# Insomnia34/charon

Measured on AMD Instinct MI355X. Metric: verified BLS partial sigs/sec (node) + threshold aggregates/sec, 1/2/4/8 GPU, higher is better.
Workload: dtype u32

## Files before the change

charon_amd/csrc/ops.h:

```cpp
#pragma once
#include "../../include/hipbls.h"
#include "fr.h"
#include "h2c.h"
#include "pairing.h"
#include "pairing_lds.h"

namespace bls {

BLS_HD BLS_CALL bool pairing_check_verify(const g1a& pk, const g2a& hm, const g2a& sig) {
  g1a P[2];
  g2a Q[2];
  bool skip[2] = {false, false};
  P[0] = pk;
  Q[0] = hm;
  P[1].x = G1_GEN_X;
  P[1].y = G1_NEG_GEN_Y;
  Q[1] = sig;
  fp12 f, e;
  miller_loop_n(f, P, Q, skip, 2);
  final_exponentiation(e, f);
  return fp12_is_one(e);
}

BLS_HD BLS_CALL int pairing_check_verify_sig(const g1a& pk, const g2a& hm, const g2a& sig) {
  g1a P1;
  P1.x = G1_GEN_X;
  P1.y = G1_NEG_GEN_Y;
  fp12 f, e;
  g2j T1;
  miller_loop_2(f, pk, hm, P1, sig, &T1);
  const bool in_g2 = g2_subgroup_from_miller(T1, sig);
  final_exponentiation(e, f);
  if (!in_g2) return HIPBLS_ERR_SIGNATURE;
  return fp12_is_one(e) ? HIPBLS_OK : HIPBLS_ERR_VERIFY;
}

#ifndef BLS_VERIFY_L_CALL
#define BLS_VERIFY_L_CALL BLS_CALL
#endif
template <int S, bool INL, bool LINES = false>
BLS_HD BLS_INLINE int pairing_check_verify_sig_l_body(const g1a& pk, const g2a& hm, const g2a& sig, const f12l<S> F,
                                                    const rl_plan* plan = nullptr) {
  g1a P1;
  P1.x = G1_GEN_X;
  P1.y = G1_NEG_GEN_Y;
  fp12 f;
  bool in_g2;
  {
    g2j T1;
    if (LINES) {
      bool done = false;
      if (rl_wave_all(plan->replay != nullptr)) {
        done = miller_loop_2_l_replay<S>(f, F, pk, sig, &T1, plan->replay, plan->seed);
        rl_count(plan->lctr, RL_CTR_HITS, done);
        rl_count(plan->lctr, RL_CTR_BAD, !done);
      }
      if (!done && rl_wave_any(plan->record != nullptr)) {
        rl_recorder rec{plan->record, plan->seed};
        miller_loop_2_l_body<S, true>(f, F, pk, hm, P1, sig, &T1, rec);
        if (plan->record) {
          rl_publish(*plan, rec.h);
          rl_count(plan->lctr, RL_CTR_PUBLISHED, true);
        }
      } else if (!done) {
        miller_loop_2_l_body<S, true>(f, F, pk, hm, P1, sig, &T1);
      }
    } else if (INL)
      miller_loop_2_l_body<S, true>(f, F, pk, hm, P1, sig, &T1);
    else
      miller_loop_2_l<S, true>(f, F, pk, hm, P1, sig, &T1);
    in_g2 = g2_subgroup_from_miller(T1, sig);
  }
  final_exp_l(f, f, F);
  if (!in_g2) return HIPBLS_ERR_SIGNATURE;
  return fp12_is_one(f) ? HIPBLS_OK : HIPBLS_ERR_VERIFY;
}
template <int S>
BLS_HD BLS_VERIFY_L_CALL int pairing_check_verify_sig_l(const g1a& pk, const g2a& hm, const g2a& sig, const f12l<S> F) {
  return pairing_check_verify_sig_l_body<S, false>(pk, hm, sig, F);
}

BLS_HD BLS_INLINE int verify_inf_status(int ds, const g2a& sig) {
  if (ds == DEC_OK) {
    g2j sj;
    jac_from_aff(sj, sig);
    if (!g2_in_subgroup(sj)) return HIPBLS_ERR_SIGNATURE;
  }
  return HIPBLS_ERR_VERIFY;
}




BLS_HD BLS_CALL void lagrange_at_zero(fr& out_plain, const int64_t* ids, int n, int i) {
  fr num, den, t, xi, xj;
  fr_from_u32(num, 1);
  fr_from_u32(den, 1);
  fr_from_i64(xi, ids[i]);
  for (int j = 0; j < n; ++j) {
    if (j == i) continue;
    fr_from_i64(xj, ids[j]);
    fr_mul(num, num, xj);
    fr_sub(t, xj, xi);
    fr_mul(den, den, t);
  }
  fr_inv(den, den);
  fr_mul(t, num, den);
  fr_to_plain(out_plain, t);
}

BLS_HD BLS_INLINE uint64_t gcd_u64(uint64_t a, uint64_t b) {
  while (b) {
    const uint64_t t = a % b;
    a = b;
    b = t;
  }
  return a;
}
BLS_HD BLS_CALL bool lagrange_small(const int64_t* ids, int t, int me, int64_t& c_me, uint64_t& L) {
  if (t < 1 || t > 16) return false;
  for (int a = 0; a < t; ++a)
    if (ids[a] > (1 << 20) || ids[a] < -(1 << 20) || ids[a] == 0) return false;
  int64_t D[16];
  uint64_t l = 1;
  for (int k = 0; k < t; ++k) {
    int64_t d = 1;
    for (int j = 0; j < t; ++j) {
      if (j == k) continue;
      if (__builtin_mul_overflow(d, ids[j] - ids[k], &d)) return false;
    }
    if (d == 0 || d == INT64_MIN) return false;
    D[k] = d;
    const uint64_t ad = d < 0 ? (uint64_t)(-d) : (uint64_t)d;
    if (__builtin_mul_overflow(l, ad / gcd_u64(l, ad), &l) || l > (uint64_t)INT64_MAX) return false;
  }
  for (int k = 0; k < t; ++k) {
    int64_t n = 1;
    for (int j = 0; j < t; ++j)
      if (j != k && __builtin_mul_overflow(n, ids[j], &n)) return false;
    const uint64_t ad = D[k] < 0 ? (uint64_t)(-D[k]) : (uint64_t)D[k];
    const int64_t f = D[k] < 0 ? -(int64_t)(l / ad) : (int64_t)(l / ad);
    int64_t c;
    if (__builtin_mul_overflow(n, f, &c) || c == INT64_MIN) return false;
    if (k == me) c_me = c;
  }
  L = l;
  return true;
}

BLS_HD BLS_INLINE void g2_mul_i64(g2j& r, const g2j& p, int64_t c) {
  jac_mul_u64(r, p, c < 0 ? (uint64_t)0 - (uint64_t)c : (uint64_t)c);
  if (c < 0) {
    g2j t = r;
    jac_neg(r, t);
  }
}

BLS_HD BLS_CALL void tagg_scale_point(g2j& out, const g2j& sj, const int64_t* ids, int t, int me) {
  int64_t c;
  uint64_t L;
  if (lagrange_small(ids, t, me, c, L)) {
    g2_mul_i64(out, sj, c);
  } else {
    fr lam;
    lagrange_at_zero(lam, ids, t, me);
    g2_mul_glv4(out, sj, lam.v);
  }
}

BLS_HD BLS_CALL bool g2_subgroup_and_mul_i64(g2j& out, const g2j& sj, int64_t c) {
  const uint64_t k = c < 0 ? (uint64_t)0 - (uint64_t)c : (uint64_t)c;
  g2j pw = sj, ax, ac;
  jac_set_inf(ax);
  jac_set_inf(ac);
  for (int i = 0; i < 64; ++i) {
    if ((X_ABS >> i) & 1ull) {
      g2j t = ax;
      jac_add(ax, t, pw);
    }
    if ((k >> i) & 1ull) {
      g2j t = ac;
      jac_add_body(ac, t, pw);
    }
    if (i < 63 && ((X_ABS | k) >> (i + 1)) != 0) {
      g2j t;
      jac_dbl_body(t, pw);
      pw = t;
    }
  }
  if (c < 0) {
    g2j t = ac;
    jac_neg(ac, t);
  }
  out = ac;
  g2j q, ps;
  jac_neg(q, ax);
  g2_psi(ps, sj);
  return jac_eq(q, ps);
}

BLS_HD BLS_CALL void tagg_unscale(g2j& acc, const int64_t* ids, int t) {
  int64_t c;
  uint64_t L;
  if (!lagrange_small(ids, t, 0, c, L) || jac_is_inf(acc)) return;
  fr lf, li, plain;
  fr_from_i64(lf, (int64_t)L);
  fr_inv(li, lf);
  fr_to_plain(plain, li);
  g2j x = acc;
  g2_mul_glv4(acc, x, plain.v);
}

BLS_HD BLS_INLINE uint64_t tagg_group_L(const int64_t* ids, int t) {
  int64_t c;
  uint64_t L;
  return lagrange_small(ids, t, 0, c, L) ? L : 1;
}
BLS_HD BLS_CALL void g1_scale_affine(g1a& pk, uint64_t L) {
  if (L <= 1) return;
  g1j pj, q;
  jac_from_aff(pj, pk);
  jac_mul_u64(q, pj, L);
  jac_to_aff(pk, q);
}

BLS_HD BLS_CALL int op_threshold_aggregate(uint8_t* out96, const uint8_t* sigs, const int64_t* ids, int t) {
  int st = t > 0 ? HIPBLS_OK : HIPBLS_ERR_COMBINE;
  for (int a = 0; a < t; ++a) {
    if (ids[a] == 0) st = HIPBLS_ERR_COMBINE;
    for (int b = a + 1; b < t; ++b)
      if (ids[a] == ids[b]) st = HIPBLS_ERR_COMBINE;
  }
  g2j acc;
  jac_set_inf(acc);
  for (int k = 0; k < t; ++k) {
    g2a s;
    const int ds = g2_decompress(s, sigs + 96 * k, true);
    if (ds == DEC_BAD) return HIPBLS_ERR_SIGNATURE;
    if (st != HIPBLS_OK || ds == DEC_INF) continue;
    g2j sj, p;
    jac_from_aff(sj, s);
    tagg_scale_point(p, sj, ids, t, k);
    g2j x = acc;
    jac_add(acc, x, p);
  }
  if (st != HIPBLS_OK) return st;
  tagg_unscale(acc, ids, t);
  g2_compress(out96, acc);
  return HIPBLS_OK;
}

BLS_HD BLS_CALL int op_verify(const uint8_t* pk48, const uint8_t* msg, uint32_t msg_len, const uint8_t* sig96) {
  g1a pk;
  const int dp = g1_decompress(pk, pk48, true);
  if (dp == DEC_BAD) return HIPBLS_ERR_PUBKEY;
  g2a sig;
  const int ds = g2_decompress(sig, sig96, false);
  if (ds == DEC_BAD) return HIPBLS_ERR_SIGNATURE;
  if (dp == DEC_INF || ds == DEC_INF) return verify_inf_status(ds, sig);
  g2j hj;
  hash_to_g2(hj, msg, msg_len, DST_POP, 43);
  g2a hm;
  jac_to_aff(hm, hj);
  return pairing_check_verify_sig(pk, hm, sig);
}

template <int S, bool INL>
BLS_HD BLS_INLINE int op_verify_l_rest(int dp, const g1a& pk, const uint8_t* msg, uint32_t msg_len,
                                       const uint8_t* sig96, const f12l<S> F) {
  if (dp == DEC_BAD) return HIPBLS_ERR_PUBKEY;
  g2a sig;
  const int ds = g2_decompress(sig, sig96, false);
  if (ds == DEC_BAD) return HIPBLS_ERR_SIGNATURE;
  if (dp == DEC_INF || ds == DEC_INF) return verify_inf_status(ds, sig);
  g2j hj;
  hash_to_g2(hj, msg, msg_len, DST_POP, 43);
  g2a hm;
  jac_to_aff(hm, hj);
  return pairing_check_verify_sig_l_body<S, INL>(pk, hm, sig, F);
}
template <int S, bool INL>
BLS_HD BLS_INLINE int op_verify_l_body(const uint8_t* pk48, const uint8_t* msg, uint32_t msg_len, const uint8_t* sig96,
                                     const f12l<S> F) {
  g1a pk;
  const int dp = g1_decompress(pk, pk48, true);
  return op_verify_l_rest<S, INL>(dp, pk, msg, msg_len, sig96, F);
}
template <int S>
BLS_HD BLS_VERIFY_L_CALL int op_verify_l(const uint8_t* pk48, const uint8_t* msg, uint32_t msg_len, const uint8_t* sig96,
                                const f12l<S> F) {
  return op_verify_l_body<S, false>(pk48, msg, msg_len, sig96, F);
}
template <int S>
BLS_HD BLS_INLINE int op_verify_l_kernel(const uint8_t* pk48, const uint8_t* msg, uint32_t msg_len, const uint8_t* sig96,
                                         const f12l<S> F) {
  return op_verify_l_body<S, true>(pk48, msg, msg_len, sig96, F);
}

BLS_HD BLS_CALL int op_sign(uint8_t* out96, const uint8_t* sk32, const uint8_t* msg, uint32_t msg_len) {
  fr sk;
  if (!fr_plain_from_be32(sk, sk32)) return HIPBLS_ERR_SECRET;
  g2j h, s;
  hash_to_g2(h, msg, msg_len, DST_POP, 43);
  g2_mul_glv4(s, h, sk.v);
  g2_compress(out96, s);
  return HIPBLS_OK;
}

BLS_HD BLS_CALL int op_sk_to_pk(uint8_t* out48, const uint8_t* sk32) {
  fr sk;
  if (!fr_plain_from_be32(sk, sk32)) return HIPBLS_ERR_SECRET;
  if (fr_is_zero(sk)) return HIPBLS_ERR_SECRET;
  g1j g, pk;
  g.x = G1_GEN_X;
  g.y = G1_GEN_Y;
  fp_set_one(g.z);
  jac_mul_limbs(pk, g, sk.v, 8);
  g1_compress(out48, pk);
  return HIPBLS_OK;
}

}
```

charon_amd/csrc/pairing_lds.h:

```cpp
#pragma once
#include "pairing.h"
#include "rootcache.h"

namespace bls {

#if defined(__HIP_DEVICE_COMPILE__)
#define BLS_LDS __attribute__((address_space(3)))
#else
#define BLS_LDS
#endif

typedef uint32_t u32x4 __attribute__((vector_size(16)));

template <int S>
struct f12l {
  BLS_LDS u32x4* p;

  BLS_HD BLS_MEMBER void ld_fp(fp& r, int g) const {
    for (int j = 0; j < 3; ++j) {
      const u32x4 q = p[(g + j) * S];
      r.v[4 * j] = q[0];
      r.v[4 * j + 1] = q[1];
      r.v[4 * j + 2] = q[2];
      r.v[4 * j + 3] = q[3];
// ... 215 lines not shown
  fp2_sub(c, s.c1, d.c1);
  F.st(4, c);
  fp2_sub(c, s.c2, d.c2);
  F.st(5, c);
}

template <class A>
BLS_HD BLS_INLINE void fp6_mul_01_fetch(fp6& r, const A& a, const fp2& b0, const fp2& b1) {
#if BLS_LAZY_FP6
  fp2 xa2, c0, c1, c2;
  fp2_mul_xi(xa2, a(2));
  fp2_mul2(c0, a(0), b0, xa2, b1);
  fp2_mul2(c1, a(0), b1, a(1), b0);
  fp2_mul2(c2, a(2), b0, a(1), b1);
  r.c0 = c0;
  r.c1 = c1;
  r.c2 = c2;
#else
  fp2 t0, t1, s0, s1, u, c0, c1, c2;
  fp2_mul(t0, a(0), b0);
  fp2_mul(t1, a(1), b1);
  fp2_mul(u, a(2), b1);
  fp2_mul_xi(u, u);
  fp2_add(c0, u, t0);
  fp2_add_lazy(s0, a(0), a(1));
  fp2_add(s1, b0, b1);
  fp2_mul(c1, s0, s1);
  fp2_sub(c1, c1, t0);
  fp2_sub(c1, c1, t1);
  fp2_mul(c2, a(2), b0);
  fp2_add(c2, c2, t1);
  r.c0 = c0;
  r.c1 = c1;
  r.c2 = c2;
#endif
}
template <class A>
BLS_HD BLS_INLINE void fp6_mul_1_fetch(fp6& r, const A& a, const fp2& b1) {
  fp2 c0;
  fp2_mul(c0, a(2), b1);
  fp2_mul_xi(r.c0, c0);
  fp2_mul(r.c1, a(0), b1);
  fp2_mul(r.c2, a(1), b1);
}

template <int S>
BLS_HD BLS_INLINE void fp12_mul_line_l(const f12l<S>& F, const fp2& g0_in, const fp2& g1_in, const fp2& h1_in) {
  const fp2 g0 = g0_in;
  const fp2 g1 = g1_in;
  const fp2 h1 = h1_in;
  fp6 t0, t1;
  fp6_mul_01_fetch(t0, [&](int i) { return F.ld(i); }, g0, g1);
  fp6_mul_1_fetch(t1, [&](int i) { return F.ld(3 + i); }, h1);
  fp2 c;
  for (int i = 0; i < 3; ++i) {
    fp2_add(c, F.ld(i), F.ld(3 + i));
    F.st(3 + i, c);
  }
  fp6 d;
  {
    fp6 vt1;
    fp6_mul_v(vt1, t1);
    fp2_add(c, t0.c0, vt1.c0);
    F.st(0, c);
    fp2_add(c, t0.c1, vt1.c1);
    F.st(1, c);
    fp2_add(c, t0.c2, vt1.c2);
    F.st(2, c);
    fp6_add(d, t0, t1);
  }
  fp2 gh1;
  fp2_add(gh1, g1, h1);
  fp6 s;
  fp6_mul_01_fetch(s, [&](int i) { return F.ld(3 + i); }, g0, gh1);
  fp2_sub(c, s.c0, d.c0);
  F.st(3, c);
  fp2_sub(c, s.c1, d.c1);
  F.st(4, c);
  fp2_sub(c, s.c2, d.c2);
  F.st(5, c);
}

#ifndef BLS_ML_PARK
#define BLS_ML_PARK 6
#endif
template <class T>
BLS_HD BLS_INLINE void park_agpr(T& x) {
#if defined(__HIP_DEVICE_COMPILE__)
  uint32_t* w = reinterpret_cast<uint32_t*>(&x);
#pragma unroll
  for (int i = 0; i < (int)(sizeof(T) / 4); ++i) asm("" : "+a"(w[i]));
#endif
}

#ifndef BLS_ML_DBL
#define BLS_ML_DBL miller_dbl_step_inl
#endif
#ifndef BLS_MILLER_L_CALL
#define BLS_MILLER_L_CALL BLS_CALL
#endif
struct rl_recorder {
  uint32_t* p;
  uint64_t h;
  BLS_HD BLS_MEMBER void put(int k, const fp2& v) {
    if (!p) return;
    rl_store_words(p + 24 * k, &v.c0.v[0], 24);
    h = rl_fold(h, &v.c0.v[0], 24);
  }
  BLS_HD BLS_MEMBER void next() {
    if (p) p += RL_LINE_WORDS;
  }
};

template <int S, bool P1_NEG_GEN = false, class SINK = line_sink_none>
BLS_HD BLS_INLINE void miller_loop_2_l_body(fp12& f_out, const f12l<S> F, const g1a& P0_in, const g2a& Q0,
                                          const g1a& P1_in, const g2a& Q1, g2j* T1_out, SINK&& sink = SINK()) {
  g1a P0 = P0_in;
  g1a P1;
  if (P1_NEG_GEN) {
    P1.x = G1_GEN_X;
    P1.y = G1_NEG_GEN_Y;
  } else {
    P1 = P1_in;
  }
  g2j T0, T1;
  T0.x = Q0.x;
  T0.y = Q0.y;
  fp2_set_one(T0.z);
  T1.x = Q1.x;
  T1.y = Q1.y;
  fp2_set_one(T1.z);
  {
    fp12 f;
    fp2 a0, a1, ah, g0, g1, h1;
    miller_dbl_step_inl(T0, a0, a1, ah, P0.x, P0.y, sink);
    sink.next();
    miller_dbl_step_inl(T1, g0, g1, h1, P1.x, P1.y);
    fp12_line_pair(f, a0, a1, ah, g0, g1, h1);
    F.st12(f);
    miller_add_step_inl(T0, a0, a1, ah, Q0, P0.x, P0.y, sink);
    sink.next();
    miller_add_step_inl(T1, g0, g1, h1, Q1, P1.x, P1.y);
    fp12_mul_line2_l(F, a0, a1, ah, g0, g1, h1);
  }
  for (int bit = 61; bit >= 0; --bit) {
#if BLS_ML_PARK & 1
    park_agpr(T0);
    park_agpr(T1);
#endif
#if BLS_ML_PARK & 4
    park_agpr(P0);
#endif
    fp12_sqr_l(F);
    fp2 a0, a1, ah, g0, g1, h1;
    BLS_ML_DBL(T0, a0, a1, ah, P0.x, P0.y, sink);
    sink.next();
#if BLS_ML_PARK & 2
    park_agpr(T0);
    park_agpr(a0);
    park_agpr(a1);
    park_agpr(ah);
#endif
    BLS_ML_DBL(T1, g0, g1, h1, P1.x, P1.y);
    fp12_mul_line2_l(F, a0, a1, ah, g0, g1, h1);
    if ((X_ABS >> bit) & 1ull) {
      miller_add_step_inl(T0, a0, a1, ah, Q0, P0.x, P0.y, sink);
      sink.next();
      miller_add_step_inl(T1, g0, g1, h1, Q1, P1.x, P1.y);
      fp12_mul_line2_l(F, a0, a1, ah, g0, g1, h1);
    }
  }
  fp12 f;
  F.ld12(f);
  fp12_conj(f_out, f);
  if (T1_out) *T1_out = T1;
}

BLS_HD BLS_INLINE void rl_line_dbl(fp2& a0, fp2& a1, fp2& ah, const uint32_t w[RL_LINE_WORDS], const g1a& P0) {
  fp2 J3, H;
  for (int k = 0; k < 12; ++k) {
    a0.c0.v[k] = w[k], a0.c1.v[k] = w[12 + k];
    J3.c0.v[k] = w[24 + k], J3.c1.v[k] = w[36 + k];
    H.c0.v[k] = w[48 + k], H.c1.v[k] = w[60 + k];
  }
  fp2_mul_fp(a1, J3, P0.x);
  fp2_mul_fp(ah, H, P0.y);
  fp2_neg(ah, ah);
}
BLS_HD BLS_INLINE void rl_line_add(fp2& a0, fp2& a1, fp2& ah, const uint32_t w[RL_LINE_WORDS], const g1a& P0) {
  fp2 theta, lambda;
  for (int k = 0; k < 12; ++k) {
    a0.c0.v[k] = w[k], a0.c1.v[k] = w[12 + k];
    theta.c0.v[k] = w[24 + k], theta.c1.v[k] = w[36 + k];
    lambda.c0.v[k] = w[48 + k], lambda.c1.v[k] = w[60 + k];
  }
  fp2_mul_fp(a1, theta, P0.x);
  fp2_neg(a1, a1);
  fp2_mul_fp(ah, lambda, P0.y);
}

template <int S>
BLS_HD BLS_INLINE bool miller_loop_2_l_replay(fp12& f_out, const f12l<S> F, const g1a& P0_in, const g2a& Q1,
                                            g2j* T1_out, const uint32_t* blk, uint64_t seed) {
  g1a P0 = P0_in;
  g1a P1;
  P1.x = G1_GEN_X;
  P1.y = G1_NEG_GEN_Y;
  g2j T1;
  T1.x = Q1.x;
  T1.y = Q1.y;
  fp2_set_one(T1.z);
  uint64_t h = seed;
  const uint32_t* p = blk;
  uint32_t chk[4];
  rl_load_check(chk, blk);
  {
    fp12 f;
    fp2 a0, a1, ah, g0, g1, h1;
    uint32_t w[RL_LINE_WORDS];
    miller_dbl_step_inl(T1, g0, g1, h1, P1.x, P1.y);
    rl_load_line(w, p);
    p += RL_LINE_WORDS;
    h = rl_fold_line(h, w);
    rl_line_dbl(a0, a1, ah, w, P0);
    fp12_line_pair(f, a0, a1, ah, g0, g1, h1);
    F.st12(f);
    miller_add_step_inl(T1, g0, g1, h1, Q1, P1.x, P1.y);
    rl_load_line(w, p);
    p += RL_LINE_WORDS;
    h = rl_fold_line(h, w);
    rl_line_add(a0, a1, ah, w, P0);
    fp12_mul_line2_l(F, a0, a1, ah, g0, g1, h1);
  }
  for (int bit = 61; bit >= 0; --bit) {
#if BLS_ML_PARK & 1
    park_agpr(T1);
#endif
#if BLS_ML_PARK & 4
    park_agpr(P0);
#endif
    fp12_sqr_l(F);
    fp2 a0, a1, ah, g0, g1, h1;
    uint32_t w[RL_LINE_WORDS];
    BLS_ML_DBL(T1, g0, g1, h1, P1.x, P1.y);
    rl_load_line(w, p);
    p += RL_LINE_WORDS;
    h = rl_fold_line(h, w);
    rl_line_dbl(a0, a1, ah, w, P0);
    fp12_mul_line2_l(F, a0, a1, ah, g0, g1, h1);
    if ((X_ABS >> bit) & 1ull) {
      miller_add_step_inl(T1, g0, g1, h1, Q1, P1.x, P1.y);
      rl_load_line(w, p);
      p += RL_LINE_WORDS;
      h = rl_fold_line(h, w);
      rl_line_add(a0, a1, ah, w, P0);
      fp12_mul_line2_l(F, a0, a1, ah, g0, g1, h1);
    }
  }
  fp12 f;
  F.ld12(f);
  fp12_conj(f_out, f);
  if (T1_out) *T1_out = T1;
  return rl_check_ok(h, chk[0], chk[1]);
}
template <int S, bool P1_NEG_GEN = false>
BLS_HD BLS_MILLER_L_CALL void miller_loop_2_l(fp12& f_out, const f12l<S> F, const g1a& P0_in, const g2a& Q0, const g1a& P1_in,
                                     const g2a& Q1, g2j* T1_out) {
  miller_loop_2_l_body<S, P1_NEG_GEN>(f_out, F, P0_in, Q0, P1_in, Q1, T1_out);
}

template <int S>
BLS_HD BLS_INLINE void fp12_mul_l(const f12l<S>& F, const fp12& b) {
  fp6 t0, t1;
  fp6_mul_fetch(t0, [&](int i) { return F.ld(i); }, [&](int i) { return i == 0 ? b.c0.c0 : (i == 1 ? b.c0.c1 : b.c0.c2); });
  fp6_mul_fetch(t1, [&](int i) { return F.ld(3 + i); }, [&](int i) { return i == 0 ? b.c1.c0 : (i == 1 ? b.c1.c1 : b.c1.c2); });
  fp2 c;
  for (int i = 0; i < 3; ++i) {
    fp2_add(c, F.ld(i), F.ld(3 + i));
    F.st(3 + i, c);
  }
  fp6 d, sb;
  {
    fp6 vt1;
    fp6_mul_v(vt1, t1);
    fp2_add(c, t0.c0, vt1.c0);
    F.st(0, c);
    fp2_add(c, t0.c1, vt1.c1);
    F.st(1, c);
    fp2_add(c, t0.c2, vt1.c2);
    F.st(2, c);
    fp6_add(d, t0, t1);
  }
  fp6_add(sb, b.c0, b.c1);
  fp6 s;
  fp6_mul_fetch(s, [&](int i) { return F.ld(3 + i); }, [&](int i) { return i == 0 ? sb.c0 : (i == 1 ? sb.c1 : sb.c2); });
  fp2_sub(c, s.c0, d.c0);
  F.st(3, c);
  fp2_sub(c, s.c1, d.c1);
  F.st(4, c);
  fp2_sub(c, s.c2, d.c2);
  F.st(5, c);
}

template <int S>
BLS_HD BLS_CALL bool fp12_cyc_exp_xabs_karabina_l(fp12& r, const fp12& a_in, const f12l<S> F) {
  static_assert(X_ABS == 0xd201000000010000ull, "the squaring counts below are |x|'s set bits");
  cyc_c st[6];
  cyc_c c;
  c.z2 = a_in.c1.c0;
  c.z3 = a_in.c0.c2;
  c.z4 = a_in.c0.c1;
  c.z5 = a_in.c1.c2;
  cyc_sqr_run(c, 16);
  st[0] = c;
  cyc_sqr_run(c, 32);
  st[1] = c;
  cyc_sqr_run(c, 9);
  st[2] = c;
  cyc_sqr_run(c, 3);
  st[3] = c;
  cyc_sqr_run(c, 2);
  st[4] = c;
  cyc_sqr_run(c, 1);
  st[5] = c;
  fp2 num[6], den[6], pre[6];
  int s;
#pragma unroll 1
  for (s = 0; s < 6; ++s) cyc_z1_parts(num[s], den[s], st[s]);
  pre[0] = den[0];
#pragma unroll 1
  for (s = 1; s < 6; ++s) fp2_mul(pre[s], pre[s - 1], den[s]);
  if (fp2_is_zero(pre[5])) return true;
  fp2 inv;
  fp2_inv(inv, pre[5]);
#pragma unroll 1
  for (s = 5; s >= 0; --s) {
    fp2 is, z1;
    if (s > 0) {
      fp2_mul(is, inv, pre[s - 1]);
      fp2_mul(inv, inv, den[s]);
    } else {
      is = inv;
    }
    fp2_mul(z1, num[s], is);
    fp12 d;
    cyc_decompress(d, st[s], z1);
    if (s == 5)
      F.st12(d);
    else
      fp12_mul_l(F, d);
  }
  F.ld12(r);
  return false;
}
template <int S>
BLS_HD BLS_INLINE void fp12_cyc_exp_xabs_l(fp12& r, const fp12& a_in, const f12l<S>& F) {
  if (fp12_cyc_exp_xabs_karabina_l(r, a_in, F)) fp12_cyc_exp_xabs_gs(r, a_in);
}

template <int S>
BLS_HD BLS_CALL void final_exponentiation_l(fp12& r, const fp12& f_in, const f12l<S> F) {
  fp12 m;
  {
    fp12 t, fi;
    fp12_conj(t, f_in);
    fp12_inv(fi, f_in);
    BLS_FE_MUL(m, t, fi);
    fp12_frobenius(t, m, 2);
    BLS_FE_MUL(m, t, m);
  }
  fp12 t1;
  {
    fp12 t0, u;
    fp12_cyc_exp_xabs_l(t0, m, F);
    BLS_FE_MUL(t0, t0, m);
    fp12_conj(t0, t0);
    fp12_cyc_exp_xabs_l(u, t0, F);
    BLS_FE_MUL(u, u, t0);
    fp12_conj(t0, u);
    fp12_cyc_exp_xabs_l(u, t0, F);
    fp12_conj(u, u);
    fp12_frobenius(t1, t0, 1);
    BLS_FE_MUL(t1, t1, u);
  }
  fp12 t2;
  {
    fp12 u;
    fp12_cyc_exp_xabs_l(u, t1, F);
    fp12_cyc_exp_xabs_l(u, u, F);
    fp12_frobenius(t2, t1, 2);
    BLS_FE_MUL(t2, t2, u);
    fp12_conj(u, t1);
    BLS_FE_MUL(t2, t2, u);
  }
  {
    fp12 u;
    fp12_cyclotomic_sqr(u, m);
    BLS_FE_MUL(u, u, m);
    BLS_FE_MUL(r, t2, u);
  }
}
#ifndef BLS_FE_LDS
#define BLS_FE_LDS 1
#endif
template <int S>
BLS_HD BLS_INLINE void final_exp_l(fp12& r, const fp12& f, const f12l<S>& F) {
#if BLS_FE_LDS
  final_exponentiation_l(r, f, F);
#else
  final_exponentiation(r, f);
#endif
}

template <int S>
BLS_HD BLS_CALL bool pairing_check_verify_l(const g1a& pk, const g2a& hm, const g2a& sig, const f12l<S> F) {
  g1a P1;
  P1.x = G1_GEN_X;
  P1.y = G1_NEG_GEN_Y;
  fp12 f;
  miller_loop_2_l<S, true>(f, F, pk, hm, P1, sig, nullptr);
  final_exp_l(f, f, F);
  return fp12_is_one(f);
}

}
```

charon_amd/csrc/tower.h:

```cpp
#pragma once
#include "field.h"

#ifndef BLS_FP6_CALL
#define BLS_FP6_CALL BLS_INLINE
#endif
#ifndef BLS_MILLER_CALL
#define BLS_MILLER_CALL BLS_INLINE
#endif

namespace bls {

struct fp6 {
  fp2 c0, c1, c2;
};
struct fp12 {
  fp6 c0, c1;
};

BLS_HD BLS_INLINE void fp2_set_zero(fp2& r) {
  fp_set_zero(r.c0);
  fp_set_zero(r.c1);
}
BLS_HD BLS_INLINE void fp2_set_one(fp2& r) {
  fp_set_one(r.c0);
  fp_set_zero(r.c1);
}
BLS_HD BLS_INLINE bool fp2_is_zero(const fp2& a) { return fp_is_zero(a.c0) && fp_is_zero(a.c1); }
BLS_HD BLS_INLINE bool fp2_eq(const fp2& a, const fp2& b) { return fp_eq(a.c0, b.c0) && fp_eq(a.c1, b.c1); }
BLS_HD BLS_INLINE void fp2_add(fp2& r, const fp2& a, const fp2& b) {
  BLS_CT_OP(CT_FP2_ADD);
  fp_add(r.c0, a.c0, b.c0);
  fp_add(r.c1, a.c1, b.c1);
}
BLS_HD BLS_INLINE void fp2_sub(fp2& r, const fp2& a, const fp2& b) {
  BLS_CT_OP(CT_FP2_SUB);
  fp_sub(r.c0, a.c0, b.c0);
  fp_sub(r.c1, a.c1, b.c1);
}
BLS_HD BLS_INLINE void fp2_neg(fp2& r, const fp2& a) {
  BLS_CT_OP(CT_FP2_NEG);
  fp_neg(r.c0, a.c0);
  fp_neg(r.c1, a.c1);
}
BLS_HD BLS_INLINE void fp2_dbl(fp2& r, const fp2& a) { fp2_add(r, a, a); }
BLS_HD BLS_INLINE void fp2_conj(fp2& r, const fp2& a) {
  r.c0 = a.c0;
  fp_neg(r.c1, a.c1);
}
#if defined(__HIP_DEVICE_COMPILE__) && BLS_FP2_PAIR
__device__ __forceinline__ void fp2p_join(fp2& r, const u32x12& c, uint32_t hm);
BLS_HD BLS_INLINE void fp2_mul_fp(fp2& r, const fp2& a, const fp& b) {
  const uint32_t hm = fp2p_mask();
  fp x, y;
#pragma unroll
  for (int j = 0; j < 12; ++j) x.v[j] = (hm & a.c1.v[j]) | (~hm & a.c0.v[j]);
  fp_mul(y, x, b);
  fp2p_join(r, fp_to_vec(y), hm);
}
#else
BLS_HD BLS_INLINE void fp2_mul_fp(fp2& r, const fp2& a, const fp& b) {
  fp_mul(r.c0, a.c0, b);
  fp_mul(r.c1, a.c1, b);
}
#endif
BLS_HD BLS_INLINE void fp2_mul_xi(fp2& r, const fp2& a) {
  fp t;
  fp_sub(t, a.c0, a.c1);
  fp_add(r.c1, a.c0, a.c1);
  r.c0 = t;
}
BLS_HD BLS_INLINE void fp2_half(fp2& r, const fp2& a) {
  fp_half(r.c0, a.c0);
  fp_half(r.c1, a.c1);
}
BLS_HD BLS_INLINE void fp2_mul_3b2(fp2& r, const fp2& a) {
  fp2 t, t4;
  fp2_mul_xi(t, a);
  fp2_add(t, t, t);
  fp2_add(t4, t, t);
  fp2_add(t, t4, t4);
  fp2_add(r, t, t4);
}
BLS_HD BLS_INLINE void fp2_mul_small(fp2& r, const fp2& a, uint32_t k) {
  fp_mul_small(r.c0, a.c0, k);
  fp_mul_small(r.c1, a.c1, k);
}


BLS_HD BLS_INLINE void fp6_set_zero(fp6& r) {
  fp2_set_zero(r.c0);
  fp2_set_zero(r.c1);
  fp2_set_zero(r.c2);
}
BLS_HD BLS_INLINE void fp6_set_one(fp6& r) {
  fp2_set_one(r.c0);
  fp2_set_zero(r.c1);
  fp2_set_zero(r.c2);
}
BLS_HD BLS_INLINE void fp6_add(fp6& r, const fp6& a, const fp6& b) {
  fp2_add(r.c0, a.c0, b.c0);
  fp2_add(r.c1, a.c1, b.c1);
  fp2_add(r.c2, a.c2, b.c2);
}
BLS_HD BLS_INLINE void fp6_sub(fp6& r, const fp6& a, const fp6& b) {
  fp2_sub(r.c0, a.c0, b.c0);
  fp2_sub(r.c1, a.c1, b.c1);
  fp2_sub(r.c2, a.c2, b.c2);
}
BLS_HD BLS_INLINE void fp6_neg(fp6& r, const fp6& a) {
  fp2_neg(r.c0, a.c0);
  fp2_neg(r.c1, a.c1);
  fp2_neg(r.c2, a.c2);
}
BLS_HD BLS_INLINE void fp6_mul_v(fp6& r, const fp6& a) {
  fp2 t;
  fp2_mul_xi(t, a.c2);
  r.c2 = a.c1;
  r.c1 = a.c0;
  r.c0 = t;
}

BLS_HD BLS_INLINE void fp12_set_one(fp12& r) {
  fp6_set_one(r.c0);
  fp6_set_zero(r.c1);
}
BLS_HD BLS_INLINE bool fp12_is_one(const fp12& a) {
  fp12 one;
  fp12_set_one(one);
  bool eq = true;
  const fp* x = &a.c0.c0.c0;
  const fp* y = &one.c0.c0.c0;
  for (int i = 0; i < 12; ++i) eq = eq && fp_eq(x[i], y[i]);
  return eq;
}
BLS_HD BLS_INLINE void fp12_conj(fp12& r, const fp12& a) {
  r.c0 = a.c0;
  fp6_neg(r.c1, a.c1);
}

#if defined(__HIP_DEVICE_COMPILE__) && BLS_FP2_PAIR
__device__ __forceinline__ void fp2p_join(fp2& r, const u32x12& c, uint32_t hm) {
  fp mine, other;
  fp_from_vec(mine, c);
#pragma unroll
  for (int j = 0; j < 12; ++j) other.v[j] = fp2p_xchg(mine.v[j]);
#pragma unroll
  for (int j = 0; j < 12; ++j) {
    r.c0.v[j] = (hm & other.v[j]) | (~hm & mine.v[j]);
    r.c1.v[j] = (hm & mine.v[j]) | (~hm & other.v[j]);
  }
}
BLS_HD BLS_INLINE void fp2_mul(fp2& r, const fp2& a, const fp2& b) {
  u32x12 a0 = fp_to_vec(a.c0), a1 = fp_to_vec(a.c1), b0 = fp_to_vec(b.c0), b1 = fp_to_vec(b.c1), c;
  uint32_t hm = fp2p_mask();
  const uint32_t h = hm;
  asm volatile(BLS_ASM_CALL("bls_fp2_mul_half_rt")
               : "+{v[0:11]}"(a0), "+{v[12:23]}"(a1), "+{v[24:35]}"(b0), "+{v[36:47]}"(b1), "={v[52:63]}"(c),
                 "+{v76}"(hm)
               : BLS_P_SGPR_IN
               : BLS_FP2_MUL_HALF_ASM_CLOBBERS, BLS_CALL_CLOBBERS);
  fp2p_join(r, c, h);
}
BLS_HD BLS_INLINE void fp2_sqr(fp2& r, const fp2& a) {
  u32x12 a0 = fp_to_vec(a.c0), a1 = fp_to_vec(a.c1), c;
  uint32_t hm = fp2p_mask();
  const uint32_t h = hm;
  asm volatile(BLS_ASM_CALL("bls_fp2_sqr_half_rt")
               : "+{v[0:11]}"(a0), "+{v[12:23]}"(a1), "={v[24:35]}"(c), "+{v76}"(hm)
               : BLS_P_SGPR_IN
               : BLS_FP2_SQR_HALF_ASM_CLOBBERS, BLS_CALL_CLOBBERS);
  fp2p_join(r, c, h);
}
#elif defined(__HIP_DEVICE_COMPILE__)
BLS_HD BLS_INLINE void fp2_mul(fp2& r, const fp2& a, const fp2& b) {
  u32x12 a0 = fp_to_vec(a.c0), a1 = fp_to_vec(a.c1), b0 = fp_to_vec(b.c0), b1 = fp_to_vec(b.c1), c0, c1;
  asm volatile(BLS_ASM_CALL("bls_fp2_mul_rt")
               : "+{v[0:11]}"(a0), "+{v[12:23]}"(a1), "+{v[24:35]}"(b0), "+{v[36:47]}"(b1), "={v[52:63]}"(c1),
                 "={v[64:75]}"(c0)
               : BLS_P_SGPR_IN
               : BLS_FP2_MUL_ASM_CLOBBERS, BLS_CALL_CLOBBERS);
  fp_from_vec(r.c0, c0);
  fp_from_vec(r.c1, c1);
}
#else
BLS_HD BLS_INLINE void fp2_mul(fp2& r, const fp2& a_in, const fp2& b_in) {
  BLS_CT_OP(CT_FP2_MUL);
#if defined(BLS_CONTRACT_CHECK)
  BLS_CONTRACT(fp_product_operand(a_in.c0) && fp_product_operand(a_in.c1) && fp_product_operand(b_in.c0) &&
                   fp_product_operand(b_in.c1),
               "fp2_mul: an operand is not below 2p and 2^382");
  g_contract_lazy_operands += !fp_canonical(a_in.c0) || !fp_canonical(a_in.c1) || !fp_canonical(b_in.c0) ||
                              !fp_canonical(b_in.c1);
  fp2 a, b;
  fp_reduce_2p(a.c0, a_in.c0);
  fp_reduce_2p(a.c1, a_in.c1);
  fp_reduce_2p(b.c0, b_in.c0);
  fp_reduce_2p(b.c1, b_in.c1);
#else
  const fp2& a = a_in;
  const fp2& b = b_in;
#endif
  fp t0, t1, t2, s0, s1;
  fp_mul(t0, a.c0, b.c0);
  fp_mul(t1, a.c1, b.c1);
  fp_add_lazy(s0, a.c0, a.c1);
  fp_add_lazy(s1, b.c0, b.c1);
  fp_mul(t2, s0, s1);
  fp_sub(r.c0, t0, t1);
  fp_sub(t2, t2, t0);
  fp_sub(r.c1, t2, t1);
}
#endif
#if defined(__HIP_DEVICE_COMPILE__) && BLS_LAZY_FP6 && !BLS_FP2_PAIR
BLS_HD BLS_INLINE void fp2_mul2(fp2& r, const fp2& x, const fp2& y, const fp2& z, const fp2& w) {
  u32x12 x0 = fp_to_vec(x.c0), x1 = fp_to_vec(x.c1), y0 = fp_to_vec(y.c0), y1 = fp_to_vec(y.c1);
  u32x12 z0 = fp_to_vec(z.c0), z1 = fp_to_vec(z.c1), w0 = fp_to_vec(w.c0), w1 = fp_to_vec(w.c1), c0, c1;
  asm volatile(BLS_ASM_CALL("bls_fp2_mul2_rt")
               : "+{v[0:11]}"(x0), "+{v[12:23]}"(x1), "+{v[24:35]}"(y0), "+{v[36:47]}"(y1), "+{v[88:99]}"(z0),
                 "+{v[100:111]}"(z1), "+{v[112:123]}"(w0), "+{v[124:135]}"(w1), "={v[52:63]}"(c1), "={v[64:75]}"(c0)
               :
               : BLS_FP2_MUL2_ASM_CLOBBERS, BLS_CALL_CLOBBERS);
  fp_from_vec(r.c0, c0);
  fp_from_vec(r.c1, c1);
}
BLS_HD BLS_INLINE void fp2_mul3(fp2& r, const fp2& x, const fp2& y, const fp2& z, const fp2& w, const fp2& u,
                                const fp2& t) {
  u32x12 x0 = fp_to_vec(x.c0), x1 = fp_to_vec(x.c1), y0 = fp_to_vec(y.c0), y1 = fp_to_vec(y.c1);
  u32x12 z0 = fp_to_vec(z.c0), z1 = fp_to_vec(z.c1), w0 = fp_to_vec(w.c0), w1 = fp_to_vec(w.c1);
  u32x12 u0 = fp_to_vec(u.c0), u1 = fp_to_vec(u.c1), t0 = fp_to_vec(t.c0), t1 = fp_to_vec(t.c1), c0, c1;
  asm volatile(BLS_ASM_CALL("bls_fp2_mul3_rt")
               : "+{v[0:11]}"(x0), "+{v[12:23]}"(x1), "+{v[24:35]}"(y0), "+{v[36:47]}"(y1), "+{v[88:99]}"(z0),
                 "+{v[100:111]}"(z1), "+{v[112:123]}"(w0), "+{v[124:135]}"(w1), "+{v[136:147]}"(u0),
                 "+{v[148:159]}"(u1), "+{v[160:171]}"(t0), "+{v[172:183]}"(t1), "={v[52:63]}"(c1), "={v[64:75]}"(c0)
               :
               : BLS_FP2_MUL2_ASM_CLOBBERS, BLS_CALL_CLOBBERS);
  fp_from_vec(r.c0, c0);
  fp_from_vec(r.c1, c1);
}
#else
BLS_HD BLS_INLINE void fp2_mul2(fp2& r, const fp2& x, const fp2& y, const fp2& z, const fp2& w) {
  fp2 a, b;
  fp2_mul(a, x, y);
  fp2_mul(b, z, w);
  fp2_add(r, a, b);
}
BLS_HD BLS_INLINE void fp2_mul3(fp2& r, const fp2& x, const fp2& y, const fp2& z, const fp2& w, const fp2& u,
                                const fp2& t) {
  fp2 a, b;
  fp2_mul2(a, x, y, z, w);
  fp2_mul(b, u, t);
  fp2_add(r, a, b);
}
#endif
BLS_HD BLS_INLINE void fp2_sqr_c(fp2& r, const fp2& a) {
  fp s, d, m;
  fp_add_lazy(s, a.c0, a.c1);
  fp_sub_lazy(d, a.c0, a.c1);
  fp_mul(m, a.c0, a.c1);
  fp_mul(r.c0, s, d);
  fp_add(r.c1, m, m);
}
#if defined(__HIP_DEVICE_COMPILE__) && BLS_FP2_PAIR
#elif defined(__HIP_DEVICE_COMPILE__)
BLS_HD BLS_INLINE void fp2_sqr(fp2& r, const fp2& a) {
  u32x12 a0 = fp_to_vec(a.c0), a1 = fp_to_vec(a.c1), c0, c1;
  asm volatile(BLS_ASM_CALL("bls_fp2_sqr_rt")
               : "+{v[0:11]}"(a0), "+{v[12:23]}"(a1), "={v[24:35]}"(c0), "={v[36:47]}"(c1)
               : BLS_P_SGPR_IN
               : BLS_FP2_SQR_ASM_CLOBBERS, BLS_CALL_CLOBBERS);
  fp_from_vec(r.c0, c0);
  fp_from_vec(r.c1, c1);
}
#else
BLS_HD BLS_INLINE void fp2_sqr(fp2& r, const fp2& a) {
  BLS_CT_OP(CT_FP2_SQR);
  BLS_CONTRACT(fp_canonical(a.c0) && fp_canonical(a.c1), "fp2_sqr: an operand is not canonical");
  fp2_sqr_c(r, a);
}
#endif
#ifndef BLS_CYC_FP2_SQR
#if BLS_FP2_PAIR
#define BLS_CYC_FP2_SQR fp2_sqr
#else
#define BLS_CYC_FP2_SQR fp2_sqr_c
#endif
#endif
BLS_HD BLS_CALL void fp2_inv(fp2& r, const fp2& a_in) {
  BLS_CT_OP(CT_FP2_INV);
  const fp2 a = a_in;
  fp t0, t1;
  fp_sqr(t0, a.c0);
  fp_sqr(t1, a.c1);
  fp_add(t0, t0, t1);
  fp_inv(t1, t0);
  fp_mul(r.c0, a.c0, t1);
  fp_mul(t0, a.c1, t1);
  fp_neg(r.c1, t0);
}

BLS_HD BLS_INLINE void fp2_add_lazy(fp2& r, const fp2& a, const fp2& b) {
  fp_add_lazy(r.c0, a.c0, b.c0);
  fp_add_lazy(r.c1, a.c1, b.c1);
}

BLS_HD BLS_FP6_CALL void fp6_mul(fp6& r, const fp6& a_in, const fp6& b_in) {
  const fp6 a = a_in, b = b_in;
  fp2 t0, t1, t2, s0, s1, u0, u1, u2;
  fp2_mul(t0, a.c0, b.c0);
  fp2_mul(t1, a.c1, b.c1);
  fp2_mul(t2, a.c2, b.c2);
  fp2_add_lazy(s0, a.c1, a.c2);
  fp2_add_lazy(s1, b.c1, b.c2);
  fp2_mul(u0, s0, s1);
  fp2_sub(u0, u0, t1);
  fp2_sub(u0, u0, t2);
  fp2_mul_xi(u0, u0);
  fp2_add(u0, u0, t0);
  fp2_add_lazy(s0, a.c0, a.c1);
  fp2_add_lazy(s1, b.c0, b.c1);
  fp2_mul(u1, s0, s1);
  fp2_sub(u1, u1, t0);
  fp2_sub(u1, u1, t1);
  fp2 x2;
  fp2_mul_xi(x2, t2);
  fp2_add(u1, u1, x2);
  fp2_add_lazy(s0, a.c0, a.c2);
  fp2_add_lazy(s1, b.c0, b.c2);
  fp2_mul(u2, s0, s1);
  fp2_sub(u2, u2, t0);
  fp2_sub(u2, u2, t2);
  fp2_add(u2, u2, t1);
  r.c0 = u0;
  r.c1 = u1;
  r.c2 = u2;
}
BLS_HD BLS_FP6_CALL void fp6_sqr(fp6& r, const fp6& a_in) {
  const fp6 a = a_in;
  fp2 s0, s1, s2, s3, s4, t;
  fp2_sqr(s0, a.c0);
  fp2_mul(s1, a.c0, a.c1);
  fp2_dbl(s1, s1);
  fp2_sub(t, a.c0, a.c1);
  fp2_add(t, t, a.c2);
  fp2_sqr(s2, t);
  fp2_mul(s3, a.c1, a.c2);
  fp2_dbl(s3, s3);
  fp2_sqr(s4, a.c2);
  fp2 c0, c1, c2;
  fp2_mul_xi(c0, s3);
  fp2_add(c0, c0, s0);
  fp2_mul_xi(c1, s4);
  fp2_add(c1, c1, s1);
  fp2_add(c2, s1, s2);
  fp2_add(c2, c2, s3);
  fp2_sub(c2, c2, s0);
  fp2_sub(c2, c2, s4);
  r.c0 = c0;
  r.c1 = c1;
  r.c2 = c2;
}
BLS_HD BLS_CALL void fp6_inv(fp6& r, const fp6& a_in) {
  const fp6 a = a_in;
  fp2 c0, c1, c2, t, s;
  fp2_sqr(c0, a.c0);
  fp2_mul(t, a.c1, a.c2);
  fp2_mul_xi(t, t);
  fp2_sub(c0, c0, t);
  fp2_sqr(c1, a.c2);
  fp2_mul_xi(c1, c1);
  fp2_mul(t, a.c0, a.c1);
  fp2_sub(c1, c1, t);
  fp2_sqr(c2, a.c1);
  fp2_mul(t, a.c0, a.c2);
  fp2_sub(c2, c2, t);
  fp2_mul(t, a.c2, c1);
  fp2_mul(s, a.c1, c2);
  fp2_add(t, t, s);
  fp2_mul_xi(t, t);
  fp2_mul(s, a.c0, c0);
  fp2_add(t, t, s);
  fp2_inv(t, t);
  fp2_mul(r.c0, c0, t);
  fp2_mul(r.c1, c1, t);
  fp2_mul(r.c2, c2, t);
}
BLS_HD BLS_FP6_CALL void fp6_mul_01(fp6& r, const fp6& a_in, const fp2& b0_in, const fp2& b1_in) {
  const fp6 a = a_in;
  const fp2 b0 = b0_in;
  const fp2 b1 = b1_in;
  fp2 t0, t1, s0, s1, u;
  fp2_mul(t0, a.c0, b0);
  fp2_mul(t1, a.c1, b1);
  fp2 c0, c1, c2;
  fp2_mul(u, a.c2, b1);
  fp2_mul_xi(u, u);
  fp2_add(c0, u, t0);
  fp2_add_lazy(s0, a.c0, a.c1);
  fp2_add(s1, b0, b1);
  fp2_mul(c1, s0, s1);
  fp2_sub(c1, c1, t0);
  fp2_sub(c1, c1, t1);
  fp2_mul(c2, a.c2, b0);
  fp2_add(c2, c2, t1);
  r.c0 = c0;
  r.c1 = c1;
  r.c2 = c2;
}
BLS_HD BLS_FP6_CALL void fp6_mul_1(fp6& r, const fp6& a_in, const fp2& b1_in) {
  const fp6 a = a_in;
  const fp2 b1 = b1_in;
  fp2 c0, c1, c2;
  fp2_mul(c0, a.c2, b1);
  fp2_mul_xi(c0, c0);
  fp2_mul(c1, a.c0, b1);
  fp2_mul(c2, a.c1, b1);
  r.c0 = c0;
  r.c1 = c1;
  r.c2 = c2;
}

#ifndef BLS_FP12_MUL_COPYIN
#define BLS_FP12_MUL_COPYIN 0
#endif
BLS_HD BLS_INLINE void fp12_mul_inl(fp12& r, const fp12& a_in, const fp12& b_in) {
#if BLS_FP12_MUL_COPYIN
  const fp12 a = a_in;
  const fp12 b = b_in;
#else
  const fp12& a = a_in;
  const fp12& b = b_in;
#endif
  fp6 t0, t1, s0, s1;
  fp6_mul(t0, a.c0, b.c0);
  fp6_mul(t1, a.c1, b.c1);
  fp6_add(s0, a.c0, a.c1);
  fp6_add(s1, b.c0, b.c1);
// ... 225 lines not shown
```

Measured before the change: 2.888 million.

## Use hybrid Karabina/GS exponentiation in final exp and optional compare-based check

The Karabina compressed-squaring exponentiation by |x| now keeps only three compressed states by default. It decompresses those three and covers the last six squarings with ordinary cyclotomic squarings, which shrinks the batched inversion and the number of decompressions. A second, compile-time option (off by default) replaces the final multiply-then-compare-to-one with an equality test of t2 against the conjugate of u. The hybrid path trades fewer inversion and decompression steps for a few extra full cyclotomic squarings, and changes register pressure.

```diff
diff --git a/charon_amd/csrc/ops.h b/charon_amd/csrc/ops.h
--- a/charon_amd/csrc/ops.h
+++ b/charon_amd/csrc/ops.h
@@ -71,9 +71,9 @@
       miller_loop_2_l<S, true>(f, F, pk, hm, P1, sig, &T1);
     in_g2 = g2_subgroup_from_miller(T1, sig);
   }
-  final_exp_l(f, f, F);
+  const bool one = final_exp_l_is_one(f, F);
   if (!in_g2) return HIPBLS_ERR_SIGNATURE;
-  return fp12_is_one(f) ? HIPBLS_OK : HIPBLS_ERR_VERIFY;
+  return one ? HIPBLS_OK : HIPBLS_ERR_VERIFY;
 }
 template <int S>
 BLS_HD BLS_VERIFY_L_CALL int pairing_check_verify_sig_l(const g1a& pk, const g2a& hm, const g2a& sig, const f12l<S> F) {
diff --git a/charon_amd/csrc/pairing_lds.h b/charon_amd/csrc/pairing_lds.h
--- a/charon_amd/csrc/pairing_lds.h
+++ b/charon_amd/csrc/pairing_lds.h
@@ -541,37 +541,53 @@
   F.st(5, c);
 }
 
-template <int S>
-BLS_HD BLS_CALL bool fp12_cyc_exp_xabs_karabina_l(fp12& r, const fp12& a_in, const f12l<S> F) {
-  static_assert(X_ABS == 0xd201000000010000ull, "the squaring counts below are |x|'s set bits");
-  cyc_c st[6];
-  cyc_c c;
-  c.z2 = a_in.c1.c0;
-  c.z3 = a_in.c0.c2;
-  c.z4 = a_in.c0.c1;
-  c.z5 = a_in.c1.c2;
-  cyc_sqr_run(c, 16);
-  st[0] = c;
-  cyc_sqr_run(c, 32);
-  st[1] = c;
-  cyc_sqr_run(c, 9);
-  st[2] = c;
-  cyc_sqr_run(c, 3);
-  st[3] = c;
-  cyc_sqr_run(c, 2);
-  st[4] = c;
-  cyc_sqr_run(c, 1);
-  st[5] = c;
-  fp2 num[6], den[6], pre[6];
+#ifndef BLS_FE_HYBRID
+#define BLS_FE_HYBRID 1
+#endif
+constexpr int KAR_STATES = BLS_FE_HYBRID ? 3 : 6;
+template <int S>
+BLS_HD BLS_INLINE bool cyc_exp_xabs_from_states_l(fp12& r, const cyc_c* st, const f12l<S>& F) {
+  fp2 num[KAR_STATES], den[KAR_STATES], pre[KAR_STATES];
   int s;
 #pragma unroll 1
-  for (s = 0; s < 6; ++s) cyc_z1_parts(num[s], den[s], st[s]);
+  for (s = 0; s < KAR_STATES; ++s) cyc_z1_parts(num[s], den[s], st[s]);
   pre[0] = den[0];
 #pragma unroll 1
-  for (s = 1; s < 6; ++s) fp2_mul(pre[s], pre[s - 1], den[s]);
-  if (fp2_is_zero(pre[5])) return true;
+  for (s = 1; s < KAR_STATES; ++s) fp2_mul(pre[s], pre[s - 1], den[s]);
+  if (fp2_is_zero(pre[KAR_STATES - 1])) return true;
   fp2 inv;
-  fp2_inv(inv, pre[5]);
+  fp2_inv(inv, pre[KAR_STATES - 1]);
+#if BLS_FE_HYBRID
+#pragma unroll 1
+  for (s = KAR_STATES - 1; s >= 0; --s) {
+    fp2 is;
+    if (s > 0) {
+      fp2_mul(is, inv, pre[s - 1]);
+      fp2_mul(inv, inv, den[s]);
+    } else {
+      is = inv;
+    }
+    fp2_mul(num[s], num[s], is);
+  }
+  fp12 d;
+#pragma unroll 1
+  for (int j = 0; j < 6; ++j) {
+    if (j < 3) {
+      cyc_decompress(d, st[j], num[j]);
+    } else {
+#pragma unroll 1
+      for (int k = j; k < 6; ++k) {
+        fp12 t;
+        fp12_cyclotomic_sqr_body(t, d);
+        d = t;
+      }
+    }
+    if (j == 0)
+      F.st12(d);
+    else
+      fp12_mul_l(F, d);
+  }
+#else
 #pragma unroll 1
   for (s = 5; s >= 0; --s) {
     fp2 is, z1;
@@ -589,16 +605,42 @@
     else
       fp12_mul_l(F, d);
   }
+#endif
   F.ld12(r);
   return false;
 }
 template <int S>
+BLS_HD BLS_CALL bool fp12_cyc_exp_xabs_karabina_l(fp12& r, const fp12& a_in, const f12l<S> F) {
+  static_assert(X_ABS == 0xd201000000010000ull, "the squaring counts below are |x|'s set bits");
+  cyc_c st[KAR_STATES];
+  cyc_c c;
+  c.z2 = a_in.c1.c0;
+  c.z3 = a_in.c0.c2;
+  c.z4 = a_in.c0.c1;
+  c.z5 = a_in.c1.c2;
+  cyc_sqr_run(c, 16);
+  st[0] = c;
+  cyc_sqr_run(c, 32);
+  st[1] = c;
+  cyc_sqr_run(c, 9);
+  st[2] = c;
+#if !BLS_FE_HYBRID
+  cyc_sqr_run(c, 3);
+  st[3] = c;
+  cyc_sqr_run(c, 2);
+  st[4] = c;
+  cyc_sqr_run(c, 1);
+  st[5] = c;
+#endif
+  return cyc_exp_xabs_from_states_l(r, st, F);
+}
+template <int S>
 BLS_HD BLS_INLINE void fp12_cyc_exp_xabs_l(fp12& r, const fp12& a_in, const f12l<S>& F) {
   if (fp12_cyc_exp_xabs_karabina_l(r, a_in, F)) fp12_cyc_exp_xabs_gs(r, a_in);
 }
 
-template <int S>
-BLS_HD BLS_CALL void final_exponentiation_l(fp12& r, const fp12& f_in, const f12l<S> F) {
+template <int S, bool CMP>
+BLS_HD BLS_INLINE bool final_exponentiation_l_body(fp12& r, const fp12& f_in, const f12l<S>& F) {
   fp12 m;
   {
     fp12 t, fi;
@@ -636,9 +678,26 @@
     fp12 u;
     fp12_cyclotomic_sqr(u, m);
     BLS_FE_MUL(u, u, m);
+    if (CMP) {
+      fp12_conj(u, u);
+      return fp12_eq(t2, u) && !fp12_is_zero(m);
+    }
     BLS_FE_MUL(r, t2, u);
   }
-}
+  return false;
+}
+template <int S>
+BLS_HD BLS_CALL void final_exponentiation_l(fp12& r, const fp12& f_in, const f12l<S> F) {
+  final_exponentiation_l_body<S, false>(r, f_in, F);
+}
+template <int S>
+BLS_HD BLS_CALL bool final_exp_is_one_l(const fp12& f_in, const f12l<S> F) {
+  fp12 unused;
+  return final_exponentiation_l_body<S, true>(unused, f_in, F);
+}
+#ifndef BLS_FE_CMP
+#define BLS_FE_CMP 0
+#endif
 #ifndef BLS_FE_LDS
 #define BLS_FE_LDS 1
 #endif
@@ -648,6 +707,15 @@
   final_exponentiation_l(r, f, F);
 #else
   final_exponentiation(r, f);
+#endif
+}
+template <int S>
+BLS_HD BLS_INLINE bool final_exp_l_is_one(fp12& f, const f12l<S>& F) {
+#if BLS_FE_LDS && BLS_FE_CMP
+  return final_exp_is_one_l(f, F);
+#else
+  final_exp_l(f, f, F);
+  return fp12_is_one(f);
 #endif
 }
 
diff --git a/charon_amd/csrc/tower.h b/charon_amd/csrc/tower.h
--- a/charon_amd/csrc/tower.h
+++ b/charon_amd/csrc/tower.h
@@ -132,6 +132,19 @@
   const fp* y = &one.c0.c0.c0;
   for (int i = 0; i < 12; ++i) eq = eq && fp_eq(x[i], y[i]);
   return eq;
+}
+BLS_HD BLS_INLINE bool fp12_eq(const fp12& a, const fp12& b) {
+  bool eq = true;
+  const fp* x = &a.c0.c0.c0;
+  const fp* y = &b.c0.c0.c0;
+  for (int i = 0; i < 12; ++i) eq = eq && fp_eq(x[i], y[i]);
+  return eq;
+}
+BLS_HD BLS_INLINE bool fp12_is_zero(const fp12& a) {
+  const fp2* x = &a.c0.c0;
+  bool z = true;
+  for (int i = 0; i < 6; ++i) z = z && fp2_is_zero(x[i]);
+  return z;
 }
 BLS_HD BLS_INLINE void fp12_conj(fp12& r, const fp12& a) {
   r.c0 = a.c0;
```

After: 2.966 million (median of 6 runs). +2.7%, better.
